# bjo5029/causal-vae

Hardware: AMD Instinct MI355X
Metric: training samples/sec on 128^3 vessel volumes (3D CausalVAE train step) (higher is better)
Workload: dtype bf16; 1 GPU; 3D vessel CausalVAE train step, 128^3 bf16 volumes (z-scored N(0,1)), batch 4/GPU, Adam lr 0.0001, ELBO = MSE-sum + 2000*MSE-sum(m) + KLD; global_batch=4, per_gpu_batch=4, parallelism=dp1, params=15346957

## Files before the change

causal_vae_amd/csrc/conv_mfma.hip:

```cpp
#include "common.h"

#ifdef CVAE_STAMP
#define CVAE_STAMP_SLOTS 32
#define CVAE_STAMP_WGS 8192
__device__ unsigned long long g_stamp[(size_t)CVAE_STAMP_WGS * CVAE_STAMP_SLOTS];
#define STAMP(i)                                                                                                         \
    do {                                                                                                                 \
        if (t == 0 && stamp_wg < CVAE_STAMP_WGS) g_stamp[(size_t)stamp_wg * CVAE_STAMP_SLOTS + (i)] = __builtin_readcyclecounter(); \
    } while (0)
#define STAMP_BEGIN()                                                                                                    \
    const unsigned stamp_wg = blockIdx.x + gridDim.x * (blockIdx.y + gridDim.y * blockIdx.z);                            \
    if (t == 0 && stamp_wg < CVAE_STAMP_WGS) {                                                                           \
        g_stamp[(size_t)stamp_wg * CVAE_STAMP_SLOTS + 30] = wall_clock64();                                              \
        g_stamp[(size_t)stamp_wg * CVAE_STAMP_SLOTS + 29] = ((unsigned long long)__builtin_amdgcn_s_getreg(63508) << 32) | __builtin_amdgcn_s_getreg(63492); \
    }                                                                                                                    \
    STAMP(0)
#define STAMP_END()                                                                                                      \
    do {                                                                                                                 \
        __builtin_amdgcn_s_waitcnt(0);                                                                                   \
        STAMP(27);                                                                                                       \
        if (t == 0 && stamp_wg < CVAE_STAMP_WGS) g_stamp[(size_t)stamp_wg * CVAE_STAMP_SLOTS + 31] = wall_clock64();     \
    } while (0)
#else
#define STAMP(i)
#define STAMP_BEGIN()
#define STAMP_END()
#endif

namespace {

CVAE_TUNABLE(BD_GS, 8);
CVAE_TUNABLE(APIPE, 3);
CVAE_TUNABLE(UPFULL_MIN_GRID, 2048);
CVAE_TUNABLE(UPFULL_MIN_WG, 512);
CVAE_TUNABLE(XPAIR_MIN_WGS, 2048);
CVAE_TUNABLE(XPAIR_2D_MIN_WGS, 512);
CVAE_TUNABLE(WG_TILES, 16);
CVAE_TUNABLE(WG_MIN_WG, 64);

struct ConvGeom {
    int B;
    int sd, sh, sw, Cs;
    int ld, lh, lw, Cl;
    int tiles_d, tiles_h, tiles_w;
};

struct f8x2 { unsigned short v; };
typedef int i32x4 __attribute__((ext_vector_type(4)));
typedef int i32x8 __attribute__((ext_vector_type(8)));
template <typename T> struct IsF8 { static constexpr bool value = false; };
template <> struct IsF8<f8x2> { static constexpr bool value = true; };
template <typename T> struct Frag;
template <> struct Frag<bf16> { bf16x8 v; };
template <> struct Frag<float> { float v[8]; };
template <> struct Frag<f8x2> { i32x4 v; };

__device__ __forceinline__ void lds_load(Frag<bf16>& f, const char* p) { f.v = *(const bf16x8*)p; }
__device__ __forceinline__ void lds_load(Frag<float>& f, const char* p) {
    const float4 a = *(const float4*)p, b = *(const float4*)(p + 16);
    f.v[0] = a.x; f.v[1] = a.y; f.v[2] = a.z; f.v[3] = a.w; f.v[4] = b.x; f.v[5] = b.y; f.v[6] = b.z; f.v[7] = b.w;
}
__device__ __forceinline__ void lds_load(Frag<f8x2>& f, const char* p) { f.v = *(const i32x4*)p; }
#define CVAE_E8M0_ONE 0x7F7F7F7F
__device__ __forceinline__ void mma(f32x16& acc, const Frag<bf16>& a, const Frag<bf16>& b) {
    acc = __builtin_amdgcn_mfma_f32_32x32x16_bf16(a.v, b.v, acc, 0, 0, 0);
}
__device__ __forceinline__ void mma(f32x16& acc, const Frag<float>& a, const Frag<float>& b) {
#pragma unroll
    for (int j = 0; j < 8; ++j) acc = __builtin_amdgcn_mfma_f32_32x32x2f32(a.v[j], b.v[j], acc, 0, 0, 0);
}
struct Frag2 { i32x8 v; };
template <typename T> struct StepFrag { using type = Frag<T>; static constexpr int PW = 1; };
template <> struct StepFrag<f8x2> { using type = Frag2; static constexpr int PW = 2; };
template <typename F>
__device__ __forceinline__ void load_step(F& f, const char* p0, const char*) { lds_load(f, p0); }
__device__ __forceinline__ void load_step(Frag2& f, const char* p0, const char* p1) {
    const i32x4 lo = *(const i32x4*)p0, hi = *(const i32x4*)p1;
    f.v = __builtin_shufflevector(lo, hi, 0, 1, 2, 3, 4, 5, 6, 7);
}
__device__ __forceinline__ void mma(f32x16& acc, const Frag2& a, const Frag2& b) {
    acc = __builtin_amdgcn_mfma_scale_f32_32x32x64_f8f6f4(a.v, b.v, acc, 0, 0, 0, CVAE_E8M0_ONE, 0, CVAE_E8M0_ONE);
}

template <int ND, int BM> struct Tile;
template <> struct Tile<3, 128> { static constexpr int TD = 4, TH = 4, TW = 8; };
template <> struct Tile<3, 256> { static constexpr int TD = 4, TH = 8, TW = 8; };
template <> struct Tile<2, 128> { static constexpr int TD = 1, TH = 8, TW = 16; };
template <> struct Tile<2, 256> { static constexpr int TD = 1, TH = 16, TW = 16; };

template <int ND> struct SubTile;
template <> struct SubTile<3> {
    static constexpr int SH = 4, SW = 8;
    __device__ static __forceinline__ int w_of(int r) { return ((r >> 2) & 1) | (((r >> 3) & 1) << 1) | ((r & 1) << 2); }
    __device__ static __forceinline__ int h_of(int r) { return ((r >> 4) & 1) | (((r >> 1) & 1) << 1); }
};
template <> struct SubTile<2> {
    static constexpr int SH = 2, SW = 16;
    __device__ static __forceinline__ int w_of(int r) { return ((r >> 2) & 1) | (((r >> 3) & 1) << 1) | ((r & 1) << 2) | (((r >> 1) & 1) << 3); }
    __device__ static __forceinline__ int h_of(int r) { return (r >> 4) & 1; }
};
template <int ND, bool UP> struct HaloPitch;
template <> struct HaloPitch<3, false> { static constexpr int RS = 10; };
template <> struct HaloPitch<3, true> { static constexpr int RS = 12; };
template <> struct HaloPitch<2, false> { static constexpr int RS = 18; };
template <> struct HaloPitch<2, true> { static constexpr int RS = 20; };

template <typename T> struct PieceW { using type = uint4; static constexpr int N = (8 * sizeof(T)) / 16; };
template <> struct PieceW<fp8> { using type = uint2; static constexpr int N = 1; };
__device__ __forceinline__ uint4 piece_sel(bool ok, uint4 v) { return make_uint4(ok ? v.x : 0u, ok ? v.y : 0u, ok ? v.z : 0u, ok ? v.w : 0u); }
__device__ __forceinline__ uint2 piece_sel(bool ok, uint2 v) { return make_uint2(ok ? v.x : 0u, ok ? v.y : 0u); }
template <typename T> struct Piece { typename PieceW<T>::type v[PieceW<T>::N]; };
template <typename T>
__device__ __forceinline__ void piece_load(Piece<T>& p, const T* src, bool ok) {
    using W = typename PieceW<T>::type;
#pragma unroll
    for (int u = 0; u < PieceW<T>::N; ++u) {
        p.v[u] = piece_sel(ok, ((const W*)src)[u]);
    }
}
template <typename T>
__device__ __forceinline__ void piece_load_raw(Piece<T>& p, const T* src) {
    using W = typename PieceW<T>::type;
#pragma unroll
    for (int u = 0; u < PieceW<T>::N; ++u) p.v[u] = ((const W*)src)[u];
}
template <typename T>
__device__ __forceinline__ void piece_store_sel(const Piece<T>& p, bool ok, char* dst) {
    using W = typename PieceW<T>::type;
#pragma unroll
    for (int u = 0; u < PieceW<T>::N; ++u) ((W*)dst)[u] = piece_sel(ok, p.v[u]);
}
template <typename T>
__device__ __forceinline__ void piece_store(const Piece<T>& p, char* dst) {
    using W = typename PieceW<T>::type;
#pragma unroll
    for (int u = 0; u < PieceW<T>::N; ++u) ((W*)dst)[u] = p.v[u];
}

__device__ __forceinline__ int xcd_remap(int b, int n) {
    const int q = n >> 3, r = n & 7, x = b & 7;
    return (x < r ? x * (q + 1) : r * (q + 1) + (x - r) * q) + (b >> 3);
}

#define CONV_GATE_PARAM_0
#define CONV_GATE_PARAM_1 , float gate_slope
#define CONV_GATE_OFF_0(x) 0.f
#define CONV_GATE_OFF_1(x) ((x) * gate_slope)
#define CONV_CAT_(a, b) a##b
#define CONV_CAT(a, b) CONV_CAT_(a, b)
#define CONV_GATE_PARAM CONV_CAT(CONV_GATE_PARAM_, CONV_GATED)
#define CONV_GATE_OFF(x) CONV_CAT(CONV_GATE_OFF_, CONV_GATED)(x)
#define CONV_GATED 0
#include "conv_data_kernel.inc"
#undef CONV_GATED
#define CONV_GATED 1
#include "conv_data_kernel.inc"
#undef CONV_GATED

#define CONV_GATED 0
#include "conv_splitk_finish_kernel.inc"
#undef CONV_GATED
#define CONV_GATED 1
#include "conv_splitk_finish_kernel.inc"
#undef CONV_GATED

struct UpVariant {
    int upfull = -1;
    int xpair = -1;
    long long walk_units = 0;
};

static int pick_ksplit(bool up, long long nwg, int nchunks) {
    if (up || nwg >= 256 || nwg < 1 || nchunks < 2) return 1;
    long long target = (512 + nwg - 1) / nwg;
    if (target > 16) target = 16;
    int best = 1;
    for (int d = 1; d <= nchunks && d <= target; ++d)
        if (nchunks % d == 0) best = d;
    return best;
}

template <typename T, int ND, bool UP, bool WIDE> struct DataForm {
    static constexpr bool KSPLIT = WIDE && (std::is_same<T, bf16>::value || (IsF8<T>::value && UP && ND == 3));
    static constexpr int WM = KSPLIT ? 1 : (WIDE ? 2 : 4), WN = WIDE ? 2 : 1, MI = KSPLIT ? 4 : 2, NI = 1, TS = KSPLIT ? 2 : 1;
    static constexpr bool BD = KSPLIT;
    static constexpr int BM = WM * MI * 32, BN = WN * NI * 32;
    static constexpr int KH_MAX = (UP && std::is_same<T, bf16>::value) ? 2 : 1;
    static int kh(const ConvGeom& g) { return (KH_MAX == 2 && g.Cs >= 128 && (g.Cs % 32) == 0) ? 2 : 1; }
    static constexpr bool XPAIR = sizeof(T) <= 2 && ((UP && ND == 3 && (TS == 2 || IsF8<T>::value)) || ND == 2);
};

struct ConvArgs {
    const void *in, *wp;
    const float* bias;
    const void* mask;
    void* out;
    ConvGeom g;
    int act;
    void* ws;
    size_t ws_bytes;
    hipStream_t stream;
    float acc_scale = 1.f, out_scale = 1.f;
    F8Side f8 = F8Side{nullptr, nullptr, nullptr};
    UpVariant var = UpVariant{};
    float gate_slope = 0.f;
};

// ... 244 lines not shown
    amax_publish_wg(slots, amx, blockIdx.x, red);
}

#define PAIR_MAX 16
struct PairTable {
    const float* w[PAIR_MAX];
    void* down[PAIR_MAX];
    void* up[PAIR_MAX];
    int Cs[PAIR_MAX], Cl[PAIR_MAX], blk_start[PAIR_MAX + 1];
    int count;
    int f8dir[PAIR_MAX];
    fp8* f8out[PAIR_MAX];
    const float* inv_scale[PAIR_MAX];
    unsigned* amax[PAIR_MAX];
};
template <typename T, int TAPS>
__global__ __launch_bounds__(256) void pack_weight_pairs_kernel(PairTable tb) {
    constexpr int TT = 16, TSPLIT = TAPS / TT, TP = TT + 1;
    __shared__ float tile[16 * 17 * TP];
    int ti = 0;
    while (ti + 1 < tb.count && (int)blockIdx.x >= tb.blk_start[ti + 1]) ++ti;
    const int Cs = tb.Cs[ti], Cl = tb.Cl[ti];
    int blk = (int)blockIdx.x - tb.blk_start[ti];
    const int tq = blk % TSPLIT; blk /= TSPLIT;
    const int nclt = Cl / 16, ncst = Cs / 16;
    const int cst = blk / nclt, clt = blk % nclt, cs0 = cst * 16, cl0 = clt * 16;
    const float* w = tb.w[ti];
    const int f8dir = tb.f8dir[ti];
    float amx = 0.f;
#pragma unroll
    for (int it = 0; it < 4; ++it) {
        const int i = threadIdx.x + it * 256, f = i & 3, cl = (i >> 2) & 15, cs = i >> 6;
        const float4 v = *(const float4*)(w + ((size_t)(cs0 + cs) * Cl + cl0 + cl) * TAPS + tq * TT + 4 * f);
        float* d = tile + (cs * 17 + cl) * TP + 4 * f;
        d[0] = v.x; d[1] = v.y; d[2] = v.z; d[3] = v.w;
        amx = fmaxf(fmaxf(amx, fmaxf(fabsf(v.x), fabsf(v.y))), fmaxf(fabsf(v.z), fabsf(v.w)));
    }
    __syncthreads();
    T* od = (T*)tb.down[ti];
    T* ou = (T*)tb.up[ti];
    const float mul8 = f8dir ? tb.inv_scale[ti][0] : 1.f;
    const int tg = threadIdx.x >> 5, e0 = (threadIdx.x & 31) * 8, a = e0 >> 4, b0 = e0 & 15;
#pragma unroll
    for (int tl = tg; tl < TT; tl += 8) {
        const int tap = tq * TT + tl;
        __attribute__((aligned(16))) T vd[8], vu[8];
#pragma unroll
        for (int q = 0; q < 8; ++q) {
            vd[q] = from_f32<T>(tile[(a * 17 + b0 + q) * TP + tl]);
            vu[q] = from_f32<T>(tile[((b0 + q) * 17 + a) * TP + tl]);
        }
        T* pd = od + ((size_t)(tap * nclt + clt) * Cs + cs0 + a) * 16 + b0;
        T* pu = ou + ((size_t)(tap * ncst + cst) * Cl + cl0 + a) * 16 + b0;
        constexpr int NU = (8 * sizeof(T)) / 16;
        if (f8dir != 1) {
#pragma unroll
            for (int u = 0; u < NU; ++u) ((uint4*)pd)[u] = ((const uint4*)vd)[u];
        }
        if (f8dir != 2) {
#pragma unroll
            for (int u = 0; u < NU; ++u) ((uint4*)pu)[u] = ((const uint4*)vu)[u];
        }
        if (f8dir) {
            float v8[8];
#pragma unroll
            for (int q = 0; q < 8; ++q) v8[q] = f8dir == 1 ? tile[(a * 17 + b0 + q) * TP + tl] : tile[((b0 + q) * 17 + a) * TP + tl];
            fp8* p8 = f8dir == 1 ? tb.f8out[ti] + ((size_t)(tap * (Cl / 32) + (cl0 >> 5)) * Cs + cs0 + a) * 32 + (cl0 & 16) + b0
                                 : tb.f8out[ti] + ((size_t)(tap * (Cs / 32) + (cs0 >> 5)) * Cl + cl0 + a) * 32 + (cs0 & 16) + b0;
            *(uint2*)p8 = pack8_fp8(v8, mul8);
        }
    }
    if (f8dir && tb.amax[ti]) {
        __syncthreads();
        amax_publish_wg(tb.amax[ti], amx, blockIdx.x, tile);
    }
}

#define WG_MULTI_MAX 8
struct WgradEntry {
    const void* S; const void* L; float* ws; float* bias_ws;
    ConvGeom g;
    int n_split, cb, tg, bias_mode;
    int xb;
    float* dW;
};
struct WgradTable { WgradEntry e[WG_MULTI_MAX]; int blk_start[WG_MULTI_MAX + 1]; int count; };

template <typename T, int ND>
__global__ __launch_bounds__(512, sizeof(T) == 2 ? 4 : 2) void conv_wgrad_kernel(WgradTable tb) {
    int ti = 0;
    while (ti + 1 < tb.count && (int)blockIdx.x >= tb.blk_start[ti + 1]) ++ti;
    const T* __restrict__ S = (const T*)tb.e[ti].S;
    const T* __restrict__ L = (const T*)tb.e[ti].L;
    float* __restrict__ ws = tb.e[ti].ws;
    float* __restrict__ bias_ws = tb.e[ti].bias_ws;
    const ConvGeom g = tb.e[ti].g;
    const int n_split = tb.e[ti].n_split, bias_mode = tb.e[ti].bias_mode, grid_y = tb.e[ti].cb;
    const int xb = (ND == 2) ? tb.e[ti].xb : 0;
    int lb = (int)blockIdx.x - tb.blk_start[ti];
    const int bx = lb % n_split; lb /= n_split;
    const int by = lb % grid_y, bz = lb / grid_y;
    using TL = Tile<ND, 128>;
    constexpr int NT = 512;
    constexpr int TD = TL::TD, TH = TL::TH, TW = TL::TW;
    constexpr int IW1 = 2 * TW + 2, IW = IW1 + (ND == 2 ? 2 : 0), IH = 2 * TH + 2;
    constexpr int SROW = 64 * sizeof(T), LROW = 32 * sizeof(T);
    constexpr int S_BYTES = 128 * SROW;
    constexpr int FB = 8 * sizeof(T);
    extern __shared__ __attribute__((aligned(16))) char smem[];
    char* s_lds = smem;
    char* l_lds = smem + S_BYTES;
    const int t = threadIdx.x, lane = t & 63, wave = t >> 6;
    const int cl_blocks = g.Cl / 32;
    const int cs0 = (by / cl_blocks) * 64, cl0 = (by % cl_blocks) * 32;
    const int kd = (ND == 3) ? bz : 0;
    const int kh = wave & 3, sg = wave >> 2;
    constexpr int LHALF = IW / 2, LPLANE = TD * IH * LHALF;
    auto s_byte = [](int m, int c) -> int { return m * SROW + ((((c >> 3) ^ (((m >> 1) & 1) << 2)) << 3) + (c & 7)) * (int)sizeof(T); };
    auto l_row = [](int line, int x) -> int { return (x & 1) * LPLANE + line * LHALF + (x >> 1); };
    const int tiles_per_b = g.tiles_d * g.tiles_h * g.tiles_w, total_tiles = (xb ? (g.B + 1) / 2 : g.B) * tiles_per_b;
    STAMP_BEGIN();
#ifdef CVAE_STAMP
    int stamp_it = 0;
#endif

    f32x16 acc[4];
#pragma unroll
    for (int k = 0; k < 4; ++k)
#pragma unroll
        for (int e = 0; e < 16; ++e) acc[k][e] = 0.f;

    const bool bias_s = bias_mode == 1 && (by % cl_blocks) == 0 && kd == 0;
    const bool bias_l = bias_mode == 2 && (by / cl_blocks) == 0 && (ND == 2 || kd == 1 || kd == 2);
    float bacc = 0.f;
    constexpr int SN = (128 * 8) / NT, MSTEP = NT / 8;
    constexpr int S_HSTEP = (MSTEP / TW) % TH, S_DSTEP = MSTEP / (TW * TH);
    static_assert(MSTEP % TW == 0 && (MSTEP / TW < TH ? MSTEP / TW : TH) - 1 + (SN - 1) * S_HSTEP < TH, "S passes step (hh, d) without carries");
    constexpr int LCP = IW * 4, LG = NT / LCP;
    constexpr int NLINES = TD * IH, LN = (NLINES + LG - 1) / LG, LN_FULL = NLINES / LG;
    static_assert(LG >= 1 && LG <= IH && LG <= 7 && LN <= 7 && IW <= 64, "lpk fields; a pass carries into d at most once");
    static_assert(((LPLANE + LG * LHALF + LHALF) * 4 + 3) * FB < 65536, "the L image offset of a thread's first line fits 16 bits");
    Piece<T> sp[SN], lp[LN];
    unsigned okmask = 0;
    const int s_sample = g.sd * g.sh * g.sw * g.Cs, l_sample = g.ld * g.lh * g.lw * g.Cl;
    unsigned lpk;
    {
        const int cp = t % LCP, lg = t / LCP, x = cp >> 2, piece = cp & 3;
        const int nl = lg < LG ? (NLINES - lg + LG - 1) / LG : 0;
        lpk = (unsigned)((l_row(lg, x) * 4 + piece) * FB) | (unsigned)x << 16 | (unsigned)piece << 22 | (unsigned)lg << 24 | (unsigned)nl << 27;
    }
    int nx_tw, nx_th, nx_td, nx_b, st_tw, st_th, st_td, st_b;
    {
        int r = bx;
        nx_tw = r % g.tiles_w; r /= g.tiles_w; nx_th = r % g.tiles_h; r /= g.tiles_h; nx_td = r % g.tiles_d; nx_b = r / g.tiles_d;
        r = n_split;
        st_tw = r % g.tiles_w; r /= g.tiles_w; st_th = r % g.tiles_h; r /= g.tiles_h; st_td = r % g.tiles_d; st_b = r / g.tiles_d;
    }
    auto load_tile = [&]() {
        const int b = nx_b * (1 + xb);
        const int o0d = nx_td * TD, o0h = nx_th * TH, o0w = nx_tw * TW;
        const T* Sb = S + (size_t)b * s_sample + cs0;
        const T* Lb = L + (size_t)b * l_sample + cl0;
        const bool b1ok = b + 1 < g.B;
        okmask = 0;
        int tz = t;
        unsigned pk = lpk;
        asm volatile("" : "+v"(tz), "+v"(pk));
        {
            const int piece = tz & 7, m0 = tz >> 3;
            const int w = m0 % TW, hh0 = m0 / TW % TH, d0 = m0 / (TW * TH);
            const int sx = (xb && w >= TW / 2) ? 1 : 0;
            const int ow = o0w + w - sx * (TW / 2);
            const bool okw = (ow < g.sw) & (!sx | b1ok);
            const unsigned cw = (unsigned)(min(ow, g.sw - 1) * g.Cs + piece * 8) + ((sx && b1ok) ? (unsigned)s_sample : 0u);
            const unsigned s_line = (unsigned)(g.sw * g.Cs);
#pragma unroll
            for (int i = 0; i < SN; ++i) {
                const int od = o0d + d0 + i * S_DSTEP, oh = o0h + hh0 + i * S_HSTEP;
                const bool ok = (od < g.sd) & (oh < g.sh) & okw;
                const unsigned off = (unsigned)(min(od, g.sd - 1) * g.sh + min(oh, g.sh - 1)) * s_line + cw;
                piece_load_raw<T>(sp[i], Sb + off);
                okmask |= (unsigned)ok << i;
            }
        }
        {
            const int x = (pk >> 16) & 63, piece = (pk >> 22) & 3, lg = (pk >> 24) & 7;
            const int sx = (xb && x >= IW / 2) ? 1 : 0;
            const int lx = 2 * o0w - 1 + x - sx * (IW / 2);
            const bool okx = ((unsigned)lx < (unsigned)g.lw) & (!sx | b1ok) & (xb | (x < IW1));
            const unsigned cx = (unsigned)(min(max(lx, 0), g.lw - 1) * g.Cl + piece * 8) + ((sx && b1ok) ? (unsigned)l_sample : 0u);
            const unsigned l_line = (unsigned)(g.lw * g.Cl);
            const int lz0 = 2 * o0d - 1 + kd, ly0 = 2 * o0h - 1;
#pragma unroll
            for (int i = 0; i < LN; ++i) {
                const int dq = (i * LG) / IH, yr = (i * LG) % IH;
                const int carry = (lg + yr >= IH) ? 1 : 0;
                const int lz = (ND == 3) ? lz0 + 2 * (dq + carry) : 0, ly = ly0 + lg + yr - carry * IH;
                const bool ok = ((unsigned)lz < (unsigned)g.ld) & ((unsigned)ly < (unsigned)g.lh) & okx;
                const unsigned off = (unsigned)(min(max(lz, 0), g.ld - 1) * g.lh + min(max(ly, 0), g.lh - 1)) * l_line + cx;
                piece_load_raw<T>(lp[i], Lb + off);
                okmask |= (unsigned)ok << (SN + i);
            }
        }
        nx_tw += st_tw;
        int carry = nx_tw >= g.tiles_w ? 1 : 0;
        nx_tw -= carry ? g.tiles_w : 0;
        nx_th += st_th + carry;
        carry = nx_th >= g.tiles_h ? 1 : 0;
        nx_th -= carry ? g.tiles_h : 0;
        nx_td += st_td + carry;
        carry = nx_td >= g.tiles_d ? 1 : 0;
        nx_td -= carry ? g.tiles_d : 0;
        nx_b += st_b + carry;
    };
    if (bx < total_tiles) load_tile();
    for (int tile = bx; tile < total_tiles; tile += n_split) {
        __syncthreads();
#ifdef CVAE_STAMP
        if (stamp_it < 8) STAMP(2 + 3 * stamp_it);
#endif
        {
            int tz = t;
            unsigned pk = lpk;
            asm volatile("" : "+v"(tz), "+v"(pk));
            char* sdst = s_lds + s_byte(tz >> 3, (tz & 7) * 8);
#pragma unroll
            for (int i = 0; i < SN; ++i) piece_store_sel<T>(sp[i], (okmask >> i) & 1, sdst + i * MSTEP * SROW);
            char* ldst = l_lds + (pk & 0xffffu);
            const int nl = (int)(pk >> 27);
            if (nl) {
#pragma unroll
                for (int i = 0; i < LN; ++i)
                    if (i < LN_FULL || nl > i) piece_store_sel<T>(lp[i], (okmask >> (SN + i)) & 1, ldst + i * LG * LHALF * LROW);
            }
        }
        __syncthreads();
#ifdef CVAE_STAMP
        if (stamp_it < 8) STAMP(3 + 3 * stamp_it);
#endif
        if (tile + n_split < total_tiles) load_tile();
        if (bias_s) {
            const int c = t & 63, pg = t >> 6;
#pragma unroll 4
            for (int j = 0; j < 16; ++j) bacc += to_f32(*(const T*)(s_lds + s_byte(pg * 16 + j, c)));
        } else if (bias_l) {
            const int c = t & 31, pg = t >> 5;
#pragma unroll 4
            for (int j = 0; j < 32; ++j) {
                const int pp = pg + 16 * j;
                const int xx = pp % (2 * TW), yy = pp / (2 * TW) % (2 * TH), dd = pp / (4 * TW * TH);
                const int xs = xx + 1 + ((xb && xx >= TW) ? 2 : 0);
                bacc += to_f32(*(const T*)(l_lds + l_row(dd * IH + yy + 1, xs) * LROW + c * (int)sizeof(T)));
            }
        }
        if constexpr (sizeof(T) == 2) {
            const int gq = lane >> 4, i16 = lane & 15, q = i16 >> 2, p = i16 & 3;
            const int hk = gq >> 1, colblk = gq & 1;
            typedef __attribute__((address_space(3))) bf16x4 lds_bf16x4;
            const char* abase[2];
            const char* bbase[2];
#pragma unroll
            for (int jj = 0; jj < 2; ++jj) {
                const int r0 = 8 * hk + 4 * jj + q;
                abase[jj] = s_lds + s_byte(r0, sg * 32 + 16 * colblk + 4 * p);
                bbase[jj] = l_lds + l_row(2 * (r0 / TW) + kh, 2 * (r0 % TW) + ((xb && (r0 % TW) >= TW / 2) ? 2 : 0)) * LROW + (16 * colblk + 4 * p) * 2;
            }
#pragma unroll
            for (int c = 0; c < 8; ++c) {
                const int hh_c = (16 * c / TW) % TH, d_c = (16 * c) / (TW * TH);
                bf16x8 a;
#pragma unroll
                for (int jj = 0; jj < 2; ++jj) {
                    const bf16x4 v = __builtin_amdgcn_ds_read_tr16_b64_v4bf16((lds_bf16x4*)(abase[jj] + 16 * c * SROW));
                    a[4 * jj + 0] = v[0]; a[4 * jj + 1] = v[1]; a[4 * jj + 2] = v[2]; a[4 * jj + 3] = v[3];
                }
#pragma unroll
                for (int kw = 0; kw < 4; ++kw) {
                    bf16x8 bv;
#pragma unroll
                    for (int jj = 0; jj < 2; ++jj) {
                        const char* bp = bbase[jj] + (((kw & 1) * LPLANE + (d_c * IH + 2 * hh_c) * LHALF + (kw >> 1)) * LROW);
                        const bf16x4 v = __builtin_amdgcn_ds_read_tr16_b64_v4bf16((lds_bf16x4*)bp);
                        bv[4 * jj + 0] = v[0]; bv[4 * jj + 1] = v[1]; bv[4 * jj + 2] = v[2]; bv[4 * jj + 3] = v[3];
                    }
                    acc[kw] = __builtin_amdgcn_mfma_f32_32x32x16_bf16(a, bv, acc[kw], 0, 0, 0);
                }
            }
        } else {
            const int r = lane & 31, hk = lane >> 5;
#pragma unroll 1
            for (int mm = 0; mm < 128; mm += 2) {
                const int m = mm + hk;
                const int w = m % TW, hh = m / TW % TH, d = m / (TW * TH);
                const int line = d * IH + 2 * hh + kh;
                const float a = *(const float*)(s_lds + s_byte(m, sg * 32 + r));
#pragma unroll
                for (int kw = 0; kw < 4; ++kw) {
                    const float bv = *(const float*)(l_lds + l_row(line, 2 * w + kw + ((xb && w >= TW / 2) ? 2 : 0)) * LROW + r * 4);
                    acc[kw] = __builtin_amdgcn_mfma_f32_32x32x2f32(a, bv, acc[kw], 0, 0, 0);
                }
            }
        }
#ifdef CVAE_STAMP
        if (stamp_it < 8) STAMP(4 + 3 * stamp_it);
        ++stamp_it;
#endif
    }
    STAMP(26);
    if (bias_s || bias_l) {
        __syncthreads();
        float* red = (float*)s_lds;
        red[t] = bacc;
        __syncthreads();
        if (bias_s && t < 64) {
            float v = 0.f;
#pragma unroll
            for (int q = 0; q < 8; ++q) v += red[q * 64 + t];
            bias_ws[((size_t)(by / cl_blocks) * n_split + bx) * 64 + t] = v;
        }
        if (bias_l && t < 32) {
            float v = 0.f;
#pragma unroll
            for (int q = 0; q < 16; ++q) v += red[q * 32 + t];
            const int half = (ND == 3) ? kd - 1 : 0, nhalf = (ND == 3) ? 2 : 1;
            bias_ws[(((size_t)(by % cl_blocks) * nhalf + half) * n_split + bx) * 32 + t] = v;
        }
    }
    const int col = lane & 31, hq = lane >> 5;
    if (float* __restrict__ dW = tb.e[ti].dW) {
        const int taps = (ND == 3) ? 64 : 16;
        float4* xch = (float4*)smem;
#pragma unroll
        for (int e0 = 0; e0 < 16; e0 += 4) {
            __syncthreads();
#pragma unroll
            for (int k = 0; k < 4; ++k)
                xch[((k * 4 + sg * 2 + hq) * 32 + col) * 4 + (kh ^ (col & 3))] = make_float4(acc[0][e0 + k] + 0.f, acc[1][e0 + k] + 0.f, acc[2][e0 + k] + 0.f, acc[3][e0 + k] + 0.f);
            __syncthreads();
#pragma unroll
            for (int k = 0; k < 4; ++k) {
                const int j = t + k * NT, khj = j & 3, clj = (j >> 2) & 31, r4 = (j >> 7) & 3, e = e0 + k;
                const int row = (r4 >> 1) * 32 + (e & 3) + 8 * (e >> 2) + 4 * (r4 & 1);
                *(float4*)(dW + ((size_t)(cs0 + row) * g.Cl + cl0 + clj) * taps + kd * 16 + khj * 4) = xch[(j & ~3) | (khj ^ (clj & 3))];
            }
        }
    } else {
        float* slab = ws + ((size_t)(bz * grid_y + by) * n_split + bx) * 32768;
#pragma unroll
        for (int e = 0; e < 16; ++e) {
            const int row = sg * 32 + (e & 3) + 8 * (e >> 2) + 4 * hq;
            *(float4*)(slab + ((kh * 64 + row) * 32 + col) * 4) = make_float4(acc[0][e], acc[1][e], acc[2][e], acc[3][e]);
        }
    }
    STAMP_END();
}

struct WgradReduceEntry {
    const float* ws; float* dW; const float* bias_ws; float* dbias;
    int Cs, Cl, n_split, cb, dw_blocks, bias_n, bias_rows, bias_width;
};
struct WgradReduceTable { WgradReduceEntry e[WG_MULTI_MAX]; int blk_start[WG_MULTI_MAX + 1]; int count, taps; };
__global__ __launch_bounds__(256) void wgrad_reduce_kernel(WgradReduceTable tb) {
    int ti = 0;
    while (ti + 1 < tb.count && (int)blockIdx.x >= tb.blk_start[ti + 1]) ++ti;
    const float* __restrict__ ws = tb.e[ti].ws;
    float* __restrict__ dW = tb.e[ti].dW;
    const float* __restrict__ bias_ws = tb.e[ti].bias_ws;
    float* __restrict__ dbias = tb.e[ti].dbias;
    const int Cl = tb.e[ti].Cl, taps = tb.taps, n_split = tb.e[ti].n_split, cb = tb.e[ti].cb, dw_blocks = tb.e[ti].dw_blocks;
    const int bias_n = tb.e[ti].bias_n, bias_rows = tb.e[ti].bias_rows, bias_width = tb.e[ti].bias_width;
    const int lbx = (int)blockIdx.x - tb.blk_start[ti];
    __shared__ float4 part[4][64];
    if (lbx >= dw_blocks) {
        __shared__ float bred[4][64];
        const int ch = (lbx - dw_blocks) * 64 + (threadIdx.x & 63), q = threadIdx.x >> 6;
        float v = 0.f;
        if (ch < bias_n) {
            const float* base = bias_ws + (size_t)(ch / bias_width) * bias_rows * bias_width + (ch % bias_width);
            for (int r = q; r < bias_rows; r += 4) v += base[(size_t)r * bias_width];
        }
        bred[q][threadIdx.x & 63] = v;
        __syncthreads();
        if (q == 0 && ch < bias_n) dbias[ch] = bred[0][threadIdx.x] + bred[1][threadIdx.x] + bred[2][threadIdx.x] + bred[3][threadIdx.x];
        return;
    }
    const int cl_blocks = Cl / 32;
    int bi = lbx;
    const int rowpair = bi % 32; bi /= 32;
    const int kh = bi % 4; bi /= 4;
    const int grp = bi;
    const int kd = grp / cb, blk = grp % cb;
    const int lane64 = threadIdx.x & 63, q = threadIdx.x >> 6;
    const int row = rowpair * 2 + (lane64 >> 5), col = lane64 & 31;
    const float* base = ws + (size_t)grp * n_split * 32768 + ((kh * 64 + row) * 32 + col) * 4;
    float4 a = make_float4(0.f, 0.f, 0.f, 0.f);
    constexpr int U = 8;
    for (int x0 = q; x0 < n_split; x0 += 4 * U) {
        float4 v[U];
#pragma unroll
        for (int u = 0; u < U; ++u) v[u] = *(const float4*)(base + (size_t)min(x0 + 4 * u, n_split - 1) * 32768);
#pragma unroll
        for (int u = 0; u < U; ++u)
            if (x0 + 4 * u < n_split) { a.x += v[u].x; a.y += v[u].y; a.z += v[u].z; a.w += v[u].w; }
    }
    part[q][lane64] = a;
    __syncthreads();
    if (q == 0) {
        const float4 b = part[1][lane64], c = part[2][lane64], d = part[3][lane64];
        a.x += b.x + c.x + d.x; a.y += b.y + c.y + d.y; a.z += b.z + c.z + d.z; a.w += b.w + c.w + d.w;
        const int cs = (blk / cl_blocks) * 64 + row, cl = (blk % cl_blocks) * 32 + col;
        *(float4*)(dW + ((size_t)cs * Cl + cl) * taps + kd * 16 + kh * 4) = a;
    }
}

#define WGRAD_MAX_WG 512
template <typename T, int ND> constexpr size_t wgrad_lds_bytes() {
    using TL = Tile<ND, 128>;
    return (size_t)128 * 64 * sizeof(T) + (size_t)TL::TD * (2 * TL::TH + 2) * (2 * TL::TW + 2 + (ND == 2 ? 2 : 0)) * 32 * sizeof(T);
}
template <typename T, int ND>
int plan_wgrad(const void* S, const void* L, float* ws, float* dW, float* dbias, int bias_mode, ConvGeom g, WgradEntry* me, WgradReduceEntry* re, int* main_blocks,
               int* reduce_blocks, long long n_split_req = 0) {
    using TL = Tile<ND, 128>;
    g.tiles_d = (g.sd + TL::TD - 1) / TL::TD; g.tiles_h = (g.sh + TL::TH - 1) / TL::TH; g.tiles_w = (g.sw + TL::TW - 1) / TL::TW;
    const int xb = (ND == 2 && g.sw <= TL::TW / 2 && g.B >= 2) ? 1 : 0;
    const long long total_tiles = (long long)(xb ? (g.B + 1) / 2 : g.B) * g.tiles_d * g.tiles_h * g.tiles_w;
    const int cb = (g.Cs / 64) * (g.Cl / 32), tg = (ND == 3) ? 4 : 1;
    long long n_split = WGRAD_MAX_WG / ((long long)cb * tg);
    long long floor_split = 256 / ((long long)cb * tg);
    if (floor_split > total_tiles) floor_split = total_tiles;
    long long by_tiles = total_tiles / 4;
    if (by_tiles < floor_split) by_tiles = floor_split;
    if (n_split > by_tiles) n_split = by_tiles;
    {
        long long req = (total_tiles + WG_TILES - 1) / WG_TILES;
        const long long groups = (long long)cb * tg;
        if (req * groups < WG_MIN_WG) req = (WG_MIN_WG + groups - 1) / groups;
        if (req < n_split) n_split = req;
    }
    if (n_split_req > 0 && n_split_req < n_split) n_split = n_split_req;
    if (n_split < 1) n_split = 1;
    if (n_split > total_tiles) n_split = total_tiles;
    if ((long long)cb * tg * n_split > (1 << 24)) return CVAE_E_BADSHAPE;
    const long long wgs = (long long)cb * tg * n_split;
    float* bias_ws = ws + (size_t)(wgs > WGRAD_MAX_WG ? wgs : WGRAD_MAX_WG) * 32768;
    if (!dbias) bias_mode = 0;
    const bool direct = n_split == 1;
    *me = WgradEntry{S, L, ws, bias_ws, g, (int)n_split, cb, tg, bias_mode, xb, direct ? dW : nullptr};
    *main_blocks = (int)wgs;
    const int dw_blocks = direct ? 0 : cb * tg * 4 * 32;
    const int bias_n = bias_mode == 1 ? g.Cs : (bias_mode == 2 ? g.Cl : 0), bias_width = bias_mode == 1 ? 64 : 32;
    const int bias_rows = (int)n_split * ((bias_mode == 2 && ND == 3) ? 2 : 1);
    *re = WgradReduceEntry{ws, dW, bias_ws, dbias, g.Cs, g.Cl, (int)n_split, cb, dw_blocks, bias_n, bias_rows, bias_width};
    *reduce_blocks = dw_blocks + (bias_n + 63) / 64;
    return CVAE_OK;
}
template <typename T, int ND>
int launch_wgrad_tables(WgradTable& mt, WgradReduceTable& rt, hipStream_t stream) {
    constexpr size_t LDS = wgrad_lds_bytes<T, ND>();
    static_assert(LDS <= CVAE_LDS_MAX, "LDS tile exceeds the 160 KiB of a CDNA4 CU");
    constexpr auto kern = conv_wgrad_kernel<T, ND>;
    if (cvae_allow_lds<kern>(LDS) != CVAE_OK) return CVAE_E_LAUNCH;
    rt.taps = (ND == 3) ? 64 : 16;
    hipLaunchKernelGGL(kern, dim3((unsigned)mt.blk_start[mt.count]), dim3(512), LDS, stream, mt);
    CVAE_CHECK_LAUNCH();
    if (rt.blk_start[rt.count] == 0) return CVAE_OK;
    hipLaunchKernelGGL(wgrad_reduce_kernel, dim3((unsigned)rt.blk_start[rt.count]), dim3(256), 0, stream, rt);
    CVAE_CHECK_LAUNCH();
    return CVAE_OK;
}
template <typename T, int ND>
int launch_wgrad(const void* S, const void* L, float* ws, float* dW, float* dbias, int bias_mode, ConvGeom g, hipStream_t stream) {
    WgradTable mt;
    WgradReduceTable rt;
    int mb, rb;
    const int rc = plan_wgrad<T, ND>(S, L, ws, dW, dbias, bias_mode, g, &mt.e[0], &rt.e[0], &mb, &rb);
    if (rc != CVAE_OK) return rc;
    mt.count = rt.count = 1;
    mt.blk_start[0] = rt.blk_start[0] = 0;
    mt.blk_start[1] = mb; rt.blk_start[1] = rb;
    return launch_wgrad_tables<T, ND>(mt, rt, stream);
}

bool geom_ok(int64_t B, int64_t sd, int64_t sh, int64_t sw, int64_t Cs, int64_t ld, int64_t lh, int64_t lw, int64_t Cl, int nd) {
    if (nd != 2 && nd != 3) return false;
    if (B < 0 || sd <= 0 || sh <= 0 || sw <= 0 || Cs <= 0 || ld <= 0 || lh <= 0 || lw <= 0 || Cl <= 0) return false;
    if (B > 65535 || sd > 32767 || sh > 32767 || sw > 32767 || ld > 65535 || lh > 65535 || lw > 65535) return false;
    if (nd == 2 && (sd != 1 || ld != 1)) return false;
    if (sd * sh * sw * Cs >= (int64_t(1) << 31) || ld * lh * lw * Cl >= (int64_t(1) << 31)) return false;
    auto pair_ok = [](int64_t s, int64_t l) { return s == l / 2; };
    if (nd == 3 && !pair_ok(sd, ld)) return false;
    return pair_ok(sh, lh) && pair_ok(sw, lw) && lh >= 2 && lw >= 2 && (nd == 2 || ld >= 2);
}

}

int cvae_conv_down_c1(const void* L, int l_dtype, const float* w, const float* bias, const void* mask, void* S, int64_t B, int64_t sd, int64_t sh, int64_t sw,
                      int64_t Cs, int64_t ld, int64_t lh, int64_t lw, int nd, int dtype, int act, hipStream_t stream, F8Side f8 = F8Side{nullptr, nullptr, nullptr});
int cvae_conv_up_c1(const void* S, const float* w, const float* bias, const void* mask, void* L, int64_t B, int64_t sd, int64_t sh, int64_t sw,
                    int64_t Cs, int64_t ld, int64_t lh, int64_t lw, int nd, int dtype, int act, hipStream_t stream, long long walk_units = 0);
int cvae_conv_up_c1_fp8in_impl(const void* S8, const float* w, const float* bias, void* L, float in_scale, int64_t B, int64_t sd, int64_t sh, int64_t sw, int64_t Cs, int act,
                               hipStream_t stream);
size_t cvae_conv_wgrad_c1_workspace_bytes(int64_t Cs, int nd);
int cvae_conv_wgrad_c1(const void* S, const void* L, int l_dtype, float* dW, float* dbias, float* dbias_l, void* workspace, size_t workspace_bytes, int64_t B, int64_t sd, int64_t sh,
                       int64_t sw, int64_t Cs, int64_t ld, int64_t lh, int64_t lw, int nd, int dtype, hipStream_t stream);

#ifdef CVAE_STAMP
extern "C" int cvae_debug_stamps(unsigned long long* host, size_t count) {
    if (count > (size_t)CVAE_STAMP_WGS * CVAE_STAMP_SLOTS) return CVAE_E_BADSHAPE;
    return hipMemcpyFromSymbol(host, HIP_SYMBOL(g_stamp), count * sizeof(unsigned long long)) == hipSuccess ? CVAE_OK : CVAE_E_LAUNCH;
}
#endif

extern "C" int cvae_conv_pack_weight(const float* w, void* packed, int64_t Cs, int64_t Cl, int nd, int for_up, int dtype, void* stream) {
    if ((nd != 2 && nd != 3) || Cs <= 0 || Cl <= 0) return CVAE_E_BADSHAPE;
    if ((!for_up && Cl % 16) || (for_up && (Cs % 16 || Cl % 32))) return CVAE_E_UNSUPPORTED;
    if (!w || !packed) return CVAE_E_NULLPTR;
    const int taps = (nd == 3) ? 64 : 16;
    const int64_t n = Cs * Cl * taps;
    return with_dtype(dtype, [&](auto tv) {
        using T = decltype(tv);
        hipLaunchKernelGGL(pack_weight_kernel<T>, dim3(cvae_grid_1d(n, 256)), dim3(256), 0, (hipStream_t)stream, w, (T*)packed, (int)Cs, (int)Cl, taps, for_up);
        return launch_rc();
    });
}

static bool fp8_pack_ok(int64_t Cs, int64_t Cl, int for_up) { return for_up ? (Cs % 32 == 0 && Cl % 32 == 0 && Cl > 1) : (Cl % 32 == 0 && Cs % 64 == 0); }
extern "C" int cvae_conv_pack_weight_pairs(const float* const* w, void* const* packed_down, void* const* packed_up, const int64_t* Cs, const int64_t* Cl,
                                           const int* f8dir, void* const* f8out, const float* const* inv_scale_dev, void* const* amax_slots,
                                           int count, int nd, int dtype, void* stream) {
    if ((nd != 2 && nd != 3) || count < 0) return CVAE_E_BADSHAPE;
// ... 413 lines not shown
```

Baseline: 5271 samples/s.

## Stage wgrad tiles with buffer loads using hardware out-of-bounds zeroing

Adds a buffered staging path to the conv weight-gradient kernel. It builds buffer resource descriptors for S and L and issues raw buffer loads, sending masked lanes to an out-of-range offset so the hardware returns zeros. This removes the per-element clamped address arithmetic and the select-on-store masking of the old path, using scalar offsets and wave ballots to compute validity. It also reworks the bias-accumulation indexing and recomputes per-entry values after the tile loop to ease register pressure. The buffered path is used only when the tensor spans fit the 32-bit record limit; otherwise the old path remains.

```diff
diff --git a/causal_vae_amd/csrc/conv_mfma.hip b/causal_vae_amd/csrc/conv_mfma.hip
--- a/causal_vae_amd/csrc/conv_mfma.hip
+++ b/causal_vae_amd/csrc/conv_mfma.hip
@@ -37,6 +37,7 @@
 CVAE_TUNABLE(XPAIR_2D_MIN_WGS, 512);
 CVAE_TUNABLE(WG_TILES, 16);
 CVAE_TUNABLE(WG_MIN_WG, 64);
+CVAE_TUNABLE(WG_BUF_SPAN, 1ll << 31);
 
 struct ConvGeom {
     int B;
@@ -123,6 +124,16 @@
     using W = typename PieceW<T>::type;
 #pragma unroll
     for (int u = 0; u < PieceW<T>::N; ++u) p.v[u] = ((const W*)src)[u];
+}
+typedef unsigned buf_u32x4 __attribute__((ext_vector_type(4)));
+template <typename T>
+__device__ __forceinline__ void piece_load_buf(Piece<T>& p, __amdgpu_buffer_rsrc_t rsrc, unsigned voff, unsigned soff) {
+    static_assert(sizeof(typename PieceW<T>::type) == 16, "16-byte words");
+#pragma unroll
+    for (int u = 0; u < PieceW<T>::N; ++u) {
+        const buf_u32x4 v = __builtin_amdgcn_raw_buffer_load_b128(rsrc, (int)(voff + 16u * u), (int)soff, 0);
+        p.v[u] = make_uint4(v.x, v.y, v.z, v.w);
+    }
 }
 template <typename T>
 __device__ __forceinline__ void piece_store_sel(const Piece<T>& p, bool ok, char* dst) {
@@ -533,9 +544,11 @@
     ConvGeom g;
     int n_split, cb, tg, bias_mode;
     int xb;
+    int bl;
     float* dW;
 };
 struct WgradTable { WgradEntry e[WG_MULTI_MAX]; int blk_start[WG_MULTI_MAX + 1]; int count; };
+template <bool BUFFERED> struct StagingForm { static constexpr bool value = BUFFERED; };
 
 template <typename T, int ND>
 __global__ __launch_bounds__(512, sizeof(T) == 2 ? 4 : 2) void conv_wgrad_kernel(WgradTable tb) {
@@ -543,8 +556,6 @@
     while (ti + 1 < tb.count && (int)blockIdx.x >= tb.blk_start[ti + 1]) ++ti;
     const T* __restrict__ S = (const T*)tb.e[ti].S;
     const T* __restrict__ L = (const T*)tb.e[ti].L;
-    float* __restrict__ ws = tb.e[ti].ws;
-    float* __restrict__ bias_ws = tb.e[ti].bias_ws;
     const ConvGeom g = tb.e[ti].g;
     const int n_split = tb.e[ti].n_split, bias_mode = tb.e[ti].bias_mode, grid_y = tb.e[ti].cb;
     const int xb = (ND == 2) ? tb.e[ti].xb : 0;
@@ -607,50 +618,116 @@
         r = n_split;
         st_tw = r % g.tiles_w; r /= g.tiles_w; st_th = r % g.tiles_h; r /= g.tiles_h; st_td = r % g.tiles_d; st_b = r / g.tiles_d;
     }
-    auto load_tile = [&]() {
+    constexpr unsigned OOB = 0x80000000u;
+    unsigned vs_own, vl_own;
+    {
+        const unsigned s_line_b = (unsigned)(g.sw * g.Cs) * (unsigned)sizeof(T), l_line_b = (unsigned)(g.lw * g.Cl) * (unsigned)sizeof(T);
+        const int piece = t & 7, m0 = t >> 3;
+        const int w = m0 % TW, hh0 = m0 / TW % TH, d0 = m0 / (TW * TH);
+        const int sx = (xb && w >= TW / 2) ? 1 : 0;
+        vs_own = (unsigned)(d0 * g.sh + hh0) * s_line_b + (unsigned)((w - sx * (TW / 2)) * g.Cs + piece * 8 + sx * s_sample) * (unsigned)sizeof(T);
+        const int cp = t % LCP, lg = t / LCP, x = cp >> 2, lpiece = cp & 3;
+        const int lsx = (xb && x >= IW / 2) ? 1 : 0;
+        vl_own = (unsigned)lg * l_line_b + (unsigned)((x - lsx * (IW / 2)) * g.Cl + lpiece * 8 + lsx * l_sample) * (unsigned)sizeof(T);
+    }
+    auto load_tile = [&](auto form) __attribute__((always_inline)) {
+        constexpr bool BL = decltype(form)::value;
         const int b = nx_b * (1 + xb);
         const int o0d = nx_td * TD, o0h = nx_th * TH, o0w = nx_tw * TW;
         const T* Sb = S + (size_t)b * s_sample + cs0;
         const T* Lb = L + (size_t)b * l_sample + cl0;
         const bool b1ok = b + 1 < g.B;
-        okmask = 0;
         int tz = t;
         unsigned pk = lpk;
         asm volatile("" : "+v"(tz), "+v"(pk));
-        {
-            const int piece = tz & 7, m0 = tz >> 3;
-            const int w = m0 % TW, hh0 = m0 / TW % TH, d0 = m0 / (TW * TH);
-            const int sx = (xb && w >= TW / 2) ? 1 : 0;
-            const int ow = o0w + w - sx * (TW / 2);
-            const bool okw = (ow < g.sw) & (!sx | b1ok);
-            const unsigned cw = (unsigned)(min(ow, g.sw - 1) * g.Cs + piece * 8) + ((sx && b1ok) ? (unsigned)s_sample : 0u);
-            const unsigned s_line = (unsigned)(g.sw * g.Cs);
-#pragma unroll
-            for (int i = 0; i < SN; ++i) {
-                const int od = o0d + d0 + i * S_DSTEP, oh = o0h + hh0 + i * S_HSTEP;
-                const bool ok = (od < g.sd) & (oh < g.sh) & okw;
-                const unsigned off = (unsigned)(min(od, g.sd - 1) * g.sh + min(oh, g.sh - 1)) * s_line + cw;
-                piece_load_raw<T>(sp[i], Sb + off);
-                okmask |= (unsigned)ok << i;
+        if constexpr (BL) {
+            const unsigned long long s_left = ((unsigned long long)(g.B - b) * s_sample - cs0) * sizeof(T), l_left = ((unsigned long long)(g.B - b) * l_sample - cl0) * sizeof(T);
+            auto records = [](unsigned long long left) -> int {
+                unsigned hi = (unsigned)(left >> 32);
+                asm volatile("" : "+s"(hi));
+                return (int)(hi ? OOB : min((unsigned)left, OOB));
+            };
+            int sw = g.sw, lw = g.lw;
+            asm volatile("" : "+s"(sw), "+s"(lw));
+            const unsigned s_lb = (unsigned)(sw * g.Cs) * (unsigned)sizeof(T), l_lb = (unsigned)(lw * g.Cl) * (unsigned)sizeof(T);
+            const __amdgpu_buffer_rsrc_t srs = __builtin_amdgcn_make_buffer_rsrc((void*)Sb, 0, records(s_left), 0x00020000);
+            const __amdgpu_buffer_rsrc_t lrs = __builtin_amdgcn_make_buffer_rsrc((void*)Lb, 0, records(l_left), 0x00020000);
+            {
+                const unsigned m0 = (unsigned)tz >> 3;
+                const int w = m0 % TW, hh0 = m0 / TW % TH, d0 = m0 / (TW * TH);
+                const int sx = (xb && w >= TW / 2) ? 1 : 0;
+                const bool okw = (o0w + w - sx * (TW / 2) < g.sw) & (!sx | b1ok);
+                const unsigned s_org = (unsigned)(o0d * g.sh + o0h) * s_lb + (unsigned)(o0w * g.Cs) * (unsigned)sizeof(T);
+#pragma unroll
+                for (int i = 0; i < SN; ++i) {
+                    const bool ok = (o0d + d0 + i * S_DSTEP < g.sd) & (o0h + hh0 + i * S_HSTEP < g.sh) & okw;
+                    piece_load_buf<T>(sp[i], srs, ok ? vs_own : OOB, s_org + (unsigned)(i * (S_DSTEP * g.sh + S_HSTEP)) * s_lb);
+                }
             }
-        }
-        {
-            const int x = (pk >> 16) & 63, piece = (pk >> 22) & 3, lg = (pk >> 24) & 7;
-            const int sx = (xb && x >= IW / 2) ? 1 : 0;
-            const int lx = 2 * o0w - 1 + x - sx * (IW / 2);
-            const bool okx = ((unsigned)lx < (unsigned)g.lw) & (!sx | b1ok) & (xb | (x < IW1));
-            const unsigned cx = (unsigned)(min(max(lx, 0), g.lw - 1) * g.Cl + piece * 8) + ((sx && b1ok) ? (unsigned)l_sample : 0u);
-            const unsigned l_line = (unsigned)(g.lw * g.Cl);
-            const int lz0 = 2 * o0d - 1 + kd, ly0 = 2 * o0h - 1;
-#pragma unroll
-            for (int i = 0; i < LN; ++i) {
-                const int dq = (i * LG) / IH, yr = (i * LG) % IH;
-                const int carry = (lg + yr >= IH) ? 1 : 0;
-                const int lz = (ND == 3) ? lz0 + 2 * (dq + carry) : 0, ly = ly0 + lg + yr - carry * IH;
-                const bool ok = ((unsigned)lz < (unsigned)g.ld) & ((unsigned)ly < (unsigned)g.lh) & okx;
-                const unsigned off = (unsigned)(min(max(lz, 0), g.ld - 1) * g.lh + min(max(ly, 0), g.lh - 1)) * l_line + cx;
-                piece_load_raw<T>(lp[i], Lb + off);
-                okmask |= (unsigned)ok << (SN + i);
+            {
+                const int x = (pk >> 16) & 63, lg = (pk >> 24) & 7, nl = (int)(pk >> 27);
+                const int sx = (xb && x >= IW / 2) ? 1 : 0;
+                const int lx = 2 * o0w - 1 + x - sx * (IW / 2);
+                const bool okx = ((unsigned)lx < (unsigned)g.lw) & (!sx | b1ok) & (xb | (x < IW1)) & (nl != 0);
+                const int lz0 = (ND == 3) ? 2 * o0d - 1 + kd : 0, ly0 = 2 * o0h - 1;
+                const int l_org = (lz0 * g.lh + ly0) * (int)l_lb + (2 * o0w - 1) * g.Cl * (int)sizeof(T);
+                const unsigned l_soff = (unsigned)max(l_org, 0);
+                const unsigned vl = vl_own + (unsigned)min(l_org, 0);
+                const unsigned dstep = (unsigned)(2 * g.lh - IH) * l_lb;
+                const int yb = ly0 + lg;
+                using lanes = unsigned long long;
+                const lanes okx_m = __builtin_amdgcn_ballot_w64(okx);
+#pragma unroll
+                for (int i = 0; i < LN; ++i) {
+                    const int dq = (i * LG) / IH, yr = (i * LG) % IH;
+                    const bool d0ok = (ND == 2) | ((unsigned)(lz0 + 2 * dq) < (unsigned)g.ld), d1ok = (unsigned)(lz0 + 2 * dq + 2) < (unsigned)g.ld;
+                    const bool may_carry = ND == 3 && yr + LG - 1 >= IH;
+                    const bool carry = may_carry && lg + yr >= IH;
+                    const lanes cm = __builtin_amdgcn_ballot_w64(carry);
+                    const lanes dm = (cm & (d1ok ? ~0ull : 0ull)) | (~cm & (d0ok ? ~0ull : 0ull));
+                    const lanes ym = __builtin_amdgcn_ballot_w64((unsigned)(yb + yr - (carry ? IH : 0)) < (unsigned)g.lh);
+                    const lanes pm = (i < LN_FULL) ? ~0ull : __builtin_amdgcn_ballot_w64(nl > i);
+                    const unsigned off = vl + (unsigned)(2 * dq * g.lh + yr) * l_lb + (carry ? dstep : 0u);
+                    piece_load_buf<T>(lp[i], lrs, __builtin_amdgcn_inverse_ballot_w64(dm & ym & pm & okx_m) ? off : OOB, l_soff);
+                }
+            }
+        } else {
+            okmask = 0;
+            {
+                const int piece = tz & 7, m0 = tz >> 3;
+                const int w = m0 % TW, hh0 = m0 / TW % TH, d0 = m0 / (TW * TH);
+                const int sx = (xb && w >= TW / 2) ? 1 : 0;
+                const int ow = o0w + w - sx * (TW / 2);
+                const bool okw = (ow < g.sw) & (!sx | b1ok);
+                const unsigned cw = (unsigned)(min(ow, g.sw - 1) * g.Cs + piece * 8) + ((sx && b1ok) ? (unsigned)s_sample : 0u);
+                const unsigned s_line = (unsigned)(g.sw * g.Cs);
+#pragma unroll
+                for (int i = 0; i < SN; ++i) {
+                    const int od = o0d + d0 + i * S_DSTEP, oh = o0h + hh0 + i * S_HSTEP;
+                    const bool ok = (od < g.sd) & (oh < g.sh) & okw;
+                    const unsigned off = (unsigned)(min(od, g.sd - 1) * g.sh + min(oh, g.sh - 1)) * s_line + cw;
+                    piece_load_raw<T>(sp[i], Sb + off);
+                    okmask |= (unsigned)ok << i;
+                }
+            }
+            {
+                const int x = (pk >> 16) & 63, piece = (pk >> 22) & 3, lg = (pk >> 24) & 7;
+                const int sx = (xb && x >= IW / 2) ? 1 : 0;
+                const int lx = 2 * o0w - 1 + x - sx * (IW / 2);
+                const bool okx = ((unsigned)lx < (unsigned)g.lw) & (!sx | b1ok) & (xb | (x < IW1));
+                const unsigned cx = (unsigned)(min(max(lx, 0), g.lw - 1) * g.Cl + piece * 8) + ((sx && b1ok) ? (unsigned)l_sample : 0u);
+                const unsigned l_line = (unsigned)(g.lw * g.Cl);
+                const int lz0 = 2 * o0d - 1 + kd, ly0 = 2 * o0h - 1;
+#pragma unroll
+                for (int i = 0; i < LN; ++i) {
+                    const int dq = (i * LG) / IH, yr = (i * LG) % IH;
+                    const int carry = (lg + yr >= IH) ? 1 : 0;
+                    const int lz = (ND == 3) ? lz0 + 2 * (dq + carry) : 0, ly = ly0 + lg + yr - carry * IH;
+                    const bool ok = ((unsigned)lz < (unsigned)g.ld) & ((unsigned)ly < (unsigned)g.lh) & okx;
+                    const unsigned off = (unsigned)(min(max(lz, 0), g.ld - 1) * g.lh + min(max(ly, 0), g.lh - 1)) * l_line + cx;
+                    piece_load_raw<T>(lp[i], Lb + off);
+                    okmask |= (unsigned)ok << (SN + i);
+                }
             }
         }
         nx_tw += st_tw;
@@ -664,32 +741,29 @@
         nx_td -= carry ? g.tiles_d : 0;
         nx_b += st_b + carry;
     };
-    if (bx < total_tiles) load_tile();
-    for (int tile = bx; tile < total_tiles; tile += n_split) {
-        __syncthreads();
-#ifdef CVAE_STAMP
-        if (stamp_it < 8) STAMP(2 + 3 * stamp_it);
-#endif
-        {
-            int tz = t;
-            unsigned pk = lpk;
-            asm volatile("" : "+v"(tz), "+v"(pk));
-            char* sdst = s_lds + s_byte(tz >> 3, (tz & 7) * 8);
-#pragma unroll
-            for (int i = 0; i < SN; ++i) piece_store_sel<T>(sp[i], (okmask >> i) & 1, sdst + i * MSTEP * SROW);
-            char* ldst = l_lds + (pk & 0xffffu);
-            const int nl = (int)(pk >> 27);
-            if (nl) {
-#pragma unroll
-                for (int i = 0; i < LN; ++i)
-                    if (i < LN_FULL || nl > i) piece_store_sel<T>(lp[i], (okmask >> (SN + i)) & 1, ldst + i * LG * LHALF * LROW);
-            }
-        }
-        __syncthreads();
-#ifdef CVAE_STAMP
-        if (stamp_it < 8) STAMP(3 + 3 * stamp_it);
-#endif
-        if (tile + n_split < total_tiles) load_tile();
+    auto store_tile = [&](auto form) __attribute__((always_inline)) {
+        constexpr bool BL = decltype(form)::value;
+        int tz = t;
+        unsigned pk = lpk;
+        asm volatile("" : "+v"(tz), "+v"(pk));
+        char* sdst = s_lds + s_byte(tz >> 3, (tz & 7) * 8);
+#pragma unroll
+        for (int i = 0; i < SN; ++i) {
+            if constexpr (BL) piece_store<T>(sp[i], sdst + i * MSTEP * SROW);
+            else piece_store_sel<T>(sp[i], (okmask >> i) & 1, sdst + i * MSTEP * SROW);
+        }
+        char* ldst = l_lds + (pk & 0xffffu);
+        const int nl = (int)(pk >> 27);
+        if (nl) {
+#pragma unroll
+            for (int i = 0; i < LN; ++i)
+                if (i < LN_FULL || nl > i) {
+                    if constexpr (BL) piece_store<T>(lp[i], ldst + i * LG * LHALF * LROW);
+                    else piece_store_sel<T>(lp[i], (okmask >> (SN + i)) & 1, ldst + i * LG * LHALF * LROW);
+                }
+        }
+    };
+    auto mma_tile = [&]() __attribute__((always_inline)) {
         if (bias_s) {
             const int c = t & 63, pg = t >> 6;
 #pragma unroll 4
@@ -698,10 +772,12 @@
             const int c = t & 31, pg = t >> 5;
 #pragma unroll 4
             for (int j = 0; j < 32; ++j) {
-                const int pp = pg + 16 * j;
-                const int xx = pp % (2 * TW), yy = pp / (2 * TW) % (2 * TH), dd = pp / (4 * TW * TH);
+                static_assert((2 * TW) % 16 == 0, "16 positions are a whole part of a line");
+                const int xx = pg + 16 * (j % (2 * TW / 16)), yy = j / (2 * TW / 16) % (2 * TH), dd = j / (2 * TW / 16) / (2 * TH);
                 const int xs = xx + 1 + ((xb && xx >= TW) ? 2 : 0);
-                bacc += to_f32(*(const T*)(l_lds + l_row(dd * IH + yy + 1, xs) * LROW + c * (int)sizeof(T)));
+                int line0 = (dd * IH + yy + 1) * LHALF;
+                asm volatile("" : "+s"(line0));
+                bacc += to_f32(*(const T*)(l_lds + ((xs & 1) * LPLANE + line0 + (xs >> 1)) * LROW + c * (int)sizeof(T)));
             }
         }
         if constexpr (sizeof(T) == 2) {
@@ -752,12 +828,43 @@
                 }
             }
         }
+    };
+    auto run_tiles = [&](auto form) __attribute__((always_inline)) {
+        if (bx < total_tiles) load_tile(form);
+        for (int tile = bx; tile < total_tiles; tile += n_split) {
+            __syncthreads();
 #ifdef CVAE_STAMP
-        if (stamp_it < 8) STAMP(4 + 3 * stamp_it);
-        ++stamp_it;
+            if (stamp_it < 8) STAMP(2 + 3 * stamp_it);
 #endif
-    }
+            store_tile(form);
+            __syncthreads();
+#ifdef CVAE_STAMP
+            if (stamp_it < 8) STAMP(3 + 3 * stamp_it);
+#endif
+            if (tile + n_split < total_tiles) load_tile(form);
+            mma_tile();
+#ifdef CVAE_STAMP
+            if (stamp_it < 8) STAMP(4 + 3 * stamp_it);
+            ++stamp_it;
+#endif
+        }
+    };
+    if (WG_BUF_SPAN > 0 && tb.e[ti].bl) run_tiles(StagingForm<true>{});
+    else run_tiles(StagingForm<false>{});
     STAMP(26);
+    int te = ti;
+    asm volatile("" : "+s"(te));
+    float* __restrict__ ws = tb.e[te].ws;
+    float* __restrict__ bias_ws = tb.e[te].bias_ws;
+    {
+    const int n_split = tb.e[te].n_split, grid_y = tb.e[te].cb, cl_blocks = tb.e[te].g.Cl / 32;
+    int lb = (int)blockIdx.x - tb.blk_start[te];
+    const int bx = lb % n_split; lb /= n_split;
+    const int by = lb % grid_y, bz = lb / grid_y;
+    const int cs0 = (by / cl_blocks) * 64, cl0 = (by % cl_blocks) * 32, kd = (ND == 3) ? bz : 0;
+    const int bias_mode = tb.e[te].bias_mode;
+    const bool bias_s = bias_mode == 1 && (by % cl_blocks) == 0 && kd == 0;
+    const bool bias_l = bias_mode == 2 && (by / cl_blocks) == 0 && (ND == 2 || kd == 1 || kd == 2);
     if (bias_s || bias_l) {
         __syncthreads();
         float* red = (float*)s_lds;
@@ -778,7 +885,7 @@
         }
     }
     const int col = lane & 31, hq = lane >> 5;
-    if (float* __restrict__ dW = tb.e[ti].dW) {
+    if (float* __restrict__ dW = tb.e[te].dW) {
         const int taps = (ND == 3) ? 64 : 16;
         float4* xch = (float4*)smem;
 #pragma unroll
@@ -802,6 +909,7 @@
             const int row = sg * 32 + (e & 3) + 8 * (e >> 2) + 4 * hq;
             *(float4*)(slab + ((kh * 64 + row) * 32 + col) * 4) = make_float4(acc[0][e], acc[1][e], acc[2][e], acc[3][e]);
         }
+    }
     }
     STAMP_END();
 }
@@ -897,7 +1005,9 @@
     float* bias_ws = ws + (size_t)(wgs > WGRAD_MAX_WG ? wgs : WGRAD_MAX_WG) * 32768;
     if (!dbias) bias_mode = 0;
     const bool direct = n_split == 1;
-    *me = WgradEntry{S, L, ws, bias_ws, g, (int)n_split, cb, tg, bias_mode, xb, direct ? dW : nullptr};
+    const long long s_span = (long long)(1 + xb) * g.sd * g.sh * g.sw * g.Cs * (long long)sizeof(T), l_span = (long long)(1 + xb) * g.ld * g.lh * g.lw * g.Cl * (long long)sizeof(T);
+    const int bl = (s_span <= WG_BUF_SPAN && l_span <= WG_BUF_SPAN && WG_BUF_SPAN <= (1ll << 31)) ? 1 : 0;
+    *me = WgradEntry{S, L, ws, bias_ws, g, (int)n_split, cb, tg, bias_mode, xb, bl, direct ? dW : nullptr};
     *main_blocks = (int)wgs;
     const int dw_blocks = direct ? 0 : cb * tg * 4 * 32;
     const int bias_n = bias_mode == 1 ? g.Cs : (bias_mode == 2 ? g.Cl : 0), bias_width = bias_mode == 1 ? 64 : 32;
```

Result: no change. 5299 samples/s, median of 6 (+0.5%).
